# Lightbrite88/Argon_Monte_Carlo

Measured on AMD Instinct MI355X. Metric: particle-steps/sec, higher is better.
Workload: dtype f64; 1 GPU; cube_1e5; geometry=cube, n_particles=100000, n_per_gpu=100000, parallelism=single GPU

## Files before the change

### argon_monte_carlo_amd/csrc/amc_api.hip

```cpp
#include <math.h>
#include <stdarg.h>
#include <stdio.h>
#include <stdlib.h>
#include <string.h>

#include <algorithm>
#include <chrono>
#include <memory>
#include <vector>
#include <new>
#include <type_traits>

#include "amc_host.h"
#include "amc_resolve_dev.h"

int amc_fail(amc_ctx *c, int code, const char *fmt, ...)
{
    char buf[512];
    va_list ap;
    va_start(ap, fmt);
    vsnprintf(buf, sizeof buf, fmt, ap);
    va_end(ap);
    if (c) c->err = buf;
    return code;
// ... 278 lines not shown
        AMC_HIP(c, dalloc(c, &c->d_cnt, 1));
        AMC_HIP(c, hipMemsetAsync(c->d_cnt, 0, sizeof(amc_dev_counters), c->stream));
        AMC_HIP(c, dalloc(c, &c->d_banks, AMC_COUNTER_BANKS));
        AMC_HIP(c, hipMemsetAsync(c->d_banks, 0, sizeof(amc_counter_bank) * AMC_COUNTER_BANKS, c->stream));
        c->out.banks = c->d_banks;
        c->out.rec = c->d_rec; c->out.cap = (unsigned)mp; c->out.cnt = c->d_cnt;
        c->out.lo = p->hist_lo; c->out.hi = p->hist_hi;
        if (p->hist_bins > 0 && p->hist_hi > p->hist_lo) {
            const int nb = p->hist_bins;
            AMC_HIP(c, dalloc(c, &c->d_hist, (size_t)4 * nb * AMC_COUNTER_BANKS));
            AMC_HIP(c, hipMemsetAsync(c->d_hist, 0, sizeof(unsigned long long) * 4 * nb * AMC_COUNTER_BANKS, c->stream));
            AMC_HIP(c, dalloc(c, &c->d_edges, (size_t)nb + 1));
            std::vector<double> ed(nb + 1);
            const double step = (p->hist_hi - p->hist_lo) / (double)nb;
            for (int k = 0; k <= nb; k++) ed[k] = p->hist_lo + (double)k * step;
            ed[nb] = p->hist_hi;
            AMC_HIP(c, hipMemcpy(c->d_edges, ed.data(), sizeof(double) * (nb + 1), hipMemcpyHostToDevice));
            c->out.nbins = nb; c->out.hist = c->d_hist; c->out.edges = c->d_edges; c->out.bin_step = step;
        }
        {
            void *hp = nullptr, *dp = nullptr;
            if (palloc(c, &hp, 256, hipHostMallocMapped) == hipSuccess && hipHostGetDevicePointer(&dp, hp, 0) == hipSuccess) {
                memset(hp, 0, 256);
                c->h_host_ncand = (volatile int *)hp;
                c->d_host_ncand = (int *)dp;
                c->h_od_stall = (volatile int *)hp + 16; c->d_od_stall_host = (int *)dp + 16;
                c->h_od_done = (volatile int *)hp + 32; c->d_od_done_host = (int *)dp + 32;
            }
            AMC_HIP(c, dalloc(c, &c->d_od, 16));
            AMC_HIP(c, hipMemsetAsync(c->d_od, 0, 16 * sizeof(int), c->stream));
        }
        if (palloc(c, &c->h_pin, (size_t)4 << 20, hipHostMallocDefault) == hipSuccess) c->h_pin_bytes = (size_t)4 << 20;
        if (getenv("AMC_DEBUG_RESOLVE")) {
            AMC_HIP(c, dalloc(c, &c->d_dbg, 128 + 128 * 512));
            AMC_HIP(c, hipMemsetAsync(c->d_dbg, 0, sizeof(long long) * (128 + 128 * 512), c->stream));
            { const long long big = 0x7fffffffffffffffLL; AMC_HIP(c, hipMemcpyAsync(c->d_dbg + 28, &big, sizeof big, hipMemcpyHostToDevice, c->stream)); }
        }
        AMC_HIP(c, hipStreamSynchronize(c->stream));
    }
    *out = guard.release();
    return AMC_OK;
}

int amc_set_stream(amc_ctx *c, void *hip_stream)
{
    if (!c) return AMC_ERR_INVALID;
    hipSetDevice(c->device);
    amc_prof_collect(c);
    if (c->stream) hipStreamSynchronize(c->stream);
    c->stream = hip_stream ? (hipStream_t)hip_stream : c->own_stream;
    return AMC_OK;
}

int amc_use_null_stream(amc_ctx *c)
{
    if (!c) return AMC_ERR_INVALID;
    hipSetDevice(c->device);
    amc_prof_collect(c);
    if (c->stream) hipStreamSynchronize(c->stream);
    c->stream = nullptr;
    return AMC_OK;
}

int amc_synchronize(amc_ctx *c)
{
    if (!c) return AMC_ERR_INVALID;
// ... 546 lines not shown
    }
    if (n_paths) *n_paths = pending;
    if (n_collisions) *n_collisions = st.n_pp;
    c->n = n_full; c->lo = 0; c->hi = n_full;
    return rc;
}

int amc_profile(amc_ctx *c, int enable)
{
    if (!c) return AMC_ERR_INVALID;
    hipSetDevice(c->device);
    amc_prof_collect(c);
    c->profiling = enable != 0;
    return AMC_OK;
}

int amc_overlap_stats(amc_ctx *c, int64_t *out)
{
    if (!c || !out) return AMC_ERR_INVALID;
    AMC_HIP(c, hipSetDevice(c->device));
    amc_dev_counters now;
    int rc = amc_read_counters(c, &now);
    if (rc) return rc;
    out[0] = c->ovl_steps; out[1] = now.n_refiled; out[2] = c->overlap_mode; out[3] = c->max_extra;
    out[4] = c->od_ordered_launches; out[5] = c->od_steps; out[6] = c->od_stalls; out[7] = c->od_stalls_last;
    return AMC_OK;
}

int amc_kernel_times(amc_ctx *c, double *total_ms, int64_t *launches)
{
    if (!c) return AMC_ERR_INVALID;
    hipSetDevice(c->device);
    amc_prof_collect(c);
    if (c->d_dbg) {
        long long h[128];
        hipMemcpy(h, c->d_dbg, sizeof h, hipMemcpyDeviceToHost);
        const double n = h[11] > 0 ? (double)h[11] : 1.0;
        fprintf(stderr, "[amc k_resolve phases, us/launch] count-left %.1f claim %.1f | rounds: collect %.1f pairs %.1f clusters>=3: sort+load %.1f emulate %.1f | overlay %.1f validate %.1f commit %.1f | rounds %.2f cand %.1f complex-members %.2f launches %lld (idle hand-over only %lld)\n",
                h[0] / n / 100.0, h[1] / n / 100.0, h[6] / n / 100.0, h[7] / n / 100.0, h[2] / n / 100.0, h[3] / n / 100.0, h[14] / n / 100.0, h[4] / n / 100.0, h[5] / n / 100.0,
                h[8] / n, h[9] / n, h[10] / n, h[11], h[12]);
        fprintf(stderr, "[amc host candidate count] %d (what the next launch plan is chosen from)\n", c->h_host_ncand ? (int)*c->h_host_ncand : -1);
        if (h[12] > 0)
            fprintf(stderr, "[amc k_resolve idle hand-over, us/launch] entry -> counts read %.2f, -> hand-over written %.2f, -> through the barrier %.2f (%lld launches)\n",
                    h[16] / (double)h[12] / 100.0, h[17] / (double)h[12] / 100.0, h[18] / (double)h[12] / 100.0, h[12]);
        {
            std::vector<long long> wv((size_t)128 * 512);
            hipMemcpy(wv.data(), c->d_dbg + 128, sizeof(long long) * wv.size(), hipMemcpyDeviceToHost);
            long long s[128] = {0}, longest = 0;
            for (int w = 0; w < 512; w++) {
                for (int e = 3; e < 128; e++) if (e != 4) s[e] += wv[(size_t)128 * w + e];
                longest = std::max(longest, wv[(size_t)128 * w + 4]);
            }
            const double nl = h[25] > 0 ? (double)h[25] : 1.0;
            static const char *cn[8] = {"pair", "3-cluster", "4+-cluster", "not owner", "pair+again", "3-cluster+again", "4+-cluster+again", "not owner+again"};
            static const char *pn[12] = {"graph", "walk", "reserve", "small: after emulate", "pair emulate | by the wave: emulate", "publish", "grid probe", "first hop", "particles", "set-up", "overlay probe", "small: prepare"};
            fprintf(stderr, "[amc k_clusters_wide] working waves %lld in %lld launches; launch span (first working wave in -> last out) %.2f us, last out -> ordered workgroup in %.2f us, longest wave ever %.2f us\n",
                    s[3], h[25], h[27] / nl / 100.0, h[26] / nl / 100.0, longest / 100.0);
            fprintf(stderr, "[three-particle path of lane 0] %lld times, %lld continued from the pair's hit; loads + slots %.2f us, emulation %.2f us\n", s[5], s[6],
                    s[7] / (double)std::max<long long>(1, s[5]) / 100.0, s[124] / (double)std::max<long long>(1, s[5]) / 100.0);
            fprintf(stderr, "[pair-wave lifetimes, 2.5 us buckets]");
            for (int k = 0; k < 8; k++) fprintf(stderr, " %lld", s[24 + k]);
            fprintf(stderr, "\n");
            for (int k = 0; k < 8; k++) {
                if (!s[16 + k]) continue;
                fprintf(stderr, "[amc k_clusters_wide %-16s %7lld waves, %5.1f us]", cn[k], s[16 + k], s[8 + k] / (double)s[16 + k] / 100.0);
                for (int e = 0; e < 12; e++) fprintf(stderr, " %s %.2f", pn[e], s[32 + 12 * k + e] / (double)s[16 + k] / 100.0);
// ... 13 lines not shown
```

### argon_monte_carlo_amd/csrc/amc_commit_dev.h

```cpp
#pragma once
#include "amc_grid_dev.h"

#define AMC_COMMIT_BLOCKS 64

struct amc_commit_args {
    amc_resolve_ctl *ctl;
    const double4 *hist;
    int *ov_head;
    const int *ev_gen;
    const rs_event *ev;
    const int4 *sl_meta;
    const int *sl_hits;
    const uint8_t *sl_moved;
    const double *sl_state;
    int *slot_of;
    int max_slots, max_hist;
    long long lo, hi;
    int count_pp;
    int defer;
    int nogrid;
    int enabled;
    const int *od_stall;
    int od_tick;
    int from_wide;
    const int *wctl;
    int *host_ncand;
};

AMC_DEV void amc_commit_part(const amc_commit_args &C, const amc_out &O, const amc_grid &G, const amc_state &S, int gtid,
                             int gstride)
{
    amc_resolve_ctl *ctl = C.ctl;
    int c_active, c_ok, c_nslots, c_nhist, c_ncand, c_nclusters = 0, c_rounds;
    if (C.from_wide) {
        const amc_resolve_ctl *wc = (const amc_resolve_ctl *)C.wctl;
        c_ncand = wc->ncand;
        c_active = c_ncand > 0;
        c_nslots = 2 * c_ncand + wc->nslots; c_nhist = 4 * c_ncand + wc->nhist;
        c_ok = !wc->ovf; c_rounds = 1;
        if (gtid == 0) {
            for (int b = 0; b < 16; b++) c_nclusters += C.wctl[32 + b];
            if (C.host_ncand) *C.host_ncand = c_ncand;
            O.cnt->cand_count = 0;
        }
    } else {
        c_active = ctl->active; c_ok = ctl->ok && !ctl->ovf; c_nslots = ctl->nslots; c_nhist = ctl->nhist;
        c_ncand = ctl->ncand; c_rounds = ctl->rounds;
        if (gtid == 0) c_nclusters = ctl->nclusters;
    }
    if (!c_active) return;
    const bool ok = c_ok != 0;
    const bool defer = ok && C.defer;
    const int ns = c_nslots < C.max_slots ? c_nslots : C.max_slots;
    const int nh = c_nhist < C.max_hist ? c_nhist : C.max_hist;
    int my_hits = 0, my_fp = 0;
    for (int s = gtid; s < ns; s += gstride) {
        const int p = C.sl_meta[s].x;
        if (ok && C.count_pp) { const int hs = C.sl_hits[s]; my_hits += hs & 0xffff; my_fp += hs >> 16; }
        if (defer || p < 0) continue;
        if (ok && C.sl_moved[s]) {
            const double *t = C.sl_state + (size_t)s * RS_SLOT_DOUBLES;
            S.x[p] = t[0]; S.y[p] = t[1]; S.z[p] = t[2]; S.vx[p] = t[3]; S.vy[p] = t[4]; S.vz[p] = t[5];
            S.d[p] = t[6]; S.dx[p] = t[7]; S.dy[p] = t[8]; S.dz[p] = t[9]; S.flag[p] = t[10] != 0.0 ? 1 : 0;
        }
        C.slot_of[p] = -1;
    }
    for (int o = 32; o > 0; o >>= 1) { my_hits += __shfl_down(my_hits, o, 64); my_fp += __shfl_down(my_fp, o, 64); }
    if ((threadIdx.x & 63) == 0 && my_hits) atomicAdd(&O.banks[amc_bank_id()].n_pp, (unsigned long long)my_hits);
    if ((threadIdx.x & 63) == 0 && my_fp) atomicAdd(&O.banks[amc_bank_id()].n_fp_errors, (unsigned long long)my_fp);
    if (ok)
        for (int e = gtid; e < nh; e += gstride) {
            const int g = C.ev_gen[e];
            if (g == 0) continue;
            const rs_event ev = C.ev[e];
            if (g != C.sl_meta[ev.slot].z) continue;
            const int owner = ev.which ? ev.i : ev.j;
            if (owner < C.lo || owner >= C.hi) continue;
            amc_emit(O, ev.phase, ev.cell, ev.i, ev.j, ev.which, ev.val[0], ev.val[1], ev.val[2], ev.val[3]);
        }
    if (!C.nogrid)
        for (int h = gtid; h < nh; h += gstride) {
            const double4 r = C.hist[h];
// ... 14 lines not shown
```

### argon_monte_carlo_amd/csrc/amc_grid_dev.h

```cpp
#pragma once
#include "amc_internal.h"

AMC_DEV int amc_clampi(int v, int lo, int hi) { return v < lo ? lo : (v > hi ? hi : v); }

AMC_DEV void amc_grid_coords(const amc_grid &G, double x, double y, double z, int &cx, int &cy, int &cz)
{
    cx = amc_clampi((int)floor((x - G.x0) * G.inv_h), 0, G.gx - 1);
    cy = amc_clampi((int)floor((y - G.y0) * G.inv_h), 0, G.gy - 1);
    cz = amc_clampi((int)floor((z - G.z0) * G.inv_h), 0, G.gz - 1);
}

AMC_DEV int amc_grid_cell(const amc_grid &G, int cx, int cy, int cz, bool *outside)
{
    if (G.uniform) return (cz * G.gy + cy) * G.gx + cx;
    const int lo = G.lay_lo[cz], n = G.lay_n[cz];
    int lx = cx - lo, ly = cy - lo;
    if (lx < 0 || lx >= n || ly < 0 || ly >= n) {
        if (outside) *outside = true;
        lx = amc_clampi(lx, 0, n - 1);
        ly = amc_clampi(ly, 0, n - 1);
    }
    return G.lay_off[cz] + ly * n + lx;
}

// ... 32 lines not shown
    const bool ox = (fx0 < 0) || (fx0 > G.gx - 1), oy = (fy0 < 0) || (fy0 > G.gy - 1), oz = (fz0 < 0) || (fz0 > G.gz - 1);
    const int x_lo = amc_clampi(cx - ((fx < t || ox) ? 1 : 0), 0, G.gx - 1), x_hi = amc_clampi(cx + ((fx > 1.0 - t || ox) ? 1 : 0), 0, G.gx - 1);
    const int y_lo = amc_clampi(cy - ((fy < t || oy) ? 1 : 0), 0, G.gy - 1), y_hi = amc_clampi(cy + ((fy > 1.0 - t || oy) ? 1 : 0), 0, G.gy - 1);
    const int z_lo = amc_clampi(cz - ((fz < t || oz) ? 1 : 0), 0, G.gz - 1), z_hi = amc_clampi(cz + ((fz > 1.0 - t || oz) ? 1 : 0), 0, G.gz - 1);
    int run = c >> 1;
    for (int kz = z_lo; kz <= z_hi; kz++) {
        int lo = 0, nn = G.gx, off;
        if (G.uniform) off = kz * G.gy * G.gx;
        else { lo = G.lay_lo[kz]; nn = G.lay_n[kz]; off = G.lay_off[kz]; }
        const int a = amc_clampi(x_lo - lo, 0, nn - 1), b = amc_clampi(x_hi - lo, 0, nn - 1);
        const int ya = amc_clampi(y_lo - lo, 0, nn - 1), yb = amc_clampi(y_hi - lo, 0, nn - 1);
        const int ny = yb - ya + 1;
        if (run < ny) {
            const int row = off + (ya + run) * nn;
            if (c & 1) return b != a ? row + b : -1;
            return row + a;
        }
        run -= ny;
    }
    return -1;
}

AMC_DEV int amc_rec_next(const amc_rec &r) { return r.next; }
AMC_DEV int amc_node_particle(const amc_lists &B, int node) { return node < B.n ? node : B.extra[node - B.n]; }
AMC_DEV void amc_rec_pos(const amc_grid &G, const amc_rec &r, double &x, double &y, double &z)
{
    x = G.x0 + (double)r.x; y = G.y0 + (double)r.y; z = G.z0 + (double)r.z;
}
AMC_DEV int amc_list_head(const amc_lists &B, int c)
{
    const unsigned long long h = B.head[c];
    return ((unsigned int)(h >> 32) == B.epoch) ? (int)(unsigned int)(h & 0xffffffffULL) : -1;
}
AMC_DEV void amc_list_insert(const amc_grid &G, const amc_lists &B, int p, double x, double y, double z, bool *outside)
{
    amc_rec r;
    r.x = (float)(x - G.x0); r.y = (float)(y - G.y0); r.z = (float)(z - G.z0);
    double rx, ry, rz;
    amc_rec_pos(G, r, rx, ry, rz);
    int cx, cy, cz;
    amc_grid_coords(G, rx, ry, rz, cx, cy, cz);
    const int c = amc_grid_cell(G, cx, cy, cz, outside);
    const unsigned long long mine = ((unsigned long long)B.epoch << 32) | (unsigned int)p;
    const unsigned long long old = atomicExch(&B.head[c], mine);
    r.next = ((unsigned int)(old >> 32) == B.epoch) ? (int)(unsigned int)(old & 0xffffffffULL) : -1;
    B.rec[p] = r;
}

AMC_DEV int amc_list_keep(const amc_grid &G, const amc_lists &B, int p, double x, double y, double z, bool full, int wave_id,
                          int count0, int c_old, int node, bool *outside, bool *overflow)
{
    amc_rec r;
    r.x = (float)(x - G.x0); r.y = (float)(y - G.y0); r.z = (float)(z - G.z0);
    double rx, ry, rz;
    amc_rec_pos(G, r, rx, ry, rz);
    int cx, cy, cz;
    amc_grid_coords(G, rx, ry, rz, cx, cy, cz);
    const int c = amc_grid_cell(G, cx, cy, cz, outside);
    if (full) {
        const unsigned long long mine = ((unsigned long long)B.epoch << 32) | (unsigned int)p;
        const unsigned long long old = atomicExch(&B.head[c], mine);
        r.next = ((unsigned int)(old >> 32) == B.epoch) ? (int)(unsigned int)(old & 0xffffffffULL) : -1;
        B.rec[p] = r;
        B.cell_of[p] = c; B.node_of[p] = p;
        return 0;
    }
    const bool mover = c != c_old;
    const unsigned long long mv = __ballot(mover);
    if (!mover) {
        typedef float v3f_ __attribute__((ext_vector_type(3)));
        v3f_ v_; v_.x = r.x; v_.y = r.y; v_.z = r.z;
        *(v3f_ *)&B.rec[node] = v_;
        return count0 + __popcll(mv);
    }
    const int lane = (int)__lane_id();
    const int idx = count0 + __popcll(mv & ((1ULL << lane) - 1ULL));
    ((float *)&B.rec[node])[0] = __int_as_float(0x7fc00000);
    if (idx >= B.wave_cap) { *overflow = true; return count0 + __popcll(mv); }
    const int e = wave_id * B.wave_cap + idx, nn = B.n + e;
// ... 8 lines not shown
```

### argon_monte_carlo_amd/csrc/amc_internal.h

```cpp
#pragma once
#include <hip/hip_runtime.h>
#include <hip/hip_ext.h>
#include <stdint.h>

#include <string>
#include <vector>

#include "amc_device.h"

#define RS_SLOT_DOUBLES 12

struct amc_state {
    double *x, *y, *z, *vx, *vy, *vz, *d, *dx, *dy, *dz;
    double *px, *py, *pz;
    uint8_t *flag;
};

struct amc_grid {
    double x0, y0, z0, h;
    double inv_h;
    int uniform;
    int gx, gy, gz;
    int ncells;
    double cr_probe;
// ... 144 lines not shown
    int *d_lay;
    amc_lists B;
    amc_lists B_buf[2];
    int *extra_buf[2];
    int *extra_count;
    int max_extra;
    amc_wev wev_buf[2];
    hipStream_t stream2;
    hipEvent_t ev_detect, ev_stream;
    unsigned int *ovl_flags;
    unsigned int ovl_tick;
    int ovl_sync_values;
    int64_t ovl_steps;
    int keep_K;
    int lists_age = -1;
    int lists_owner;
    int overlap_mode;
    amc_resolve_ws W;
    char *w_slab;
    char *s_slab;
    amc_temp_ws T;
    amc_temp_dev_ws TD;
    amc_fields_ws F;
    bool allpairs;
    bool detect_ap;
    amc_out out;
    amc_path_record *d_rec;
    unsigned long long *d_hist;
    double *d_edges;
    amc_dev_counters *d_cnt;
    amc_counter_bank *d_banks;
    amc_dev_counters h_prev;
    long long *d_dbg;
    int cw_blocks_env;
    int stream_bs;
    int detect_bs;
    bool temp_unfused;
    bool overlap_split;
    bool profiling;
    double k_ms[AMC_K_COUNT];
    int64_t k_launches[AMC_K_COUNT];
    std::vector<std::pair<hipEvent_t, hipEvent_t>> ev_pool;
    std::vector<std::pair<int, int>> ev_pending;
    size_t ev_used;
    hipEvent_t prof_ev0, prof_ev1;
    bool mg_count_pp = true;
    volatile int *h_host_ncand;
    int *d_host_ncand;
    bool lazy_pending;
    bool commit_pending;
    bool commit_defer;
    unsigned int sweep_epoch;
    bool plan_split;
    int plan_small = AMC_PLAN_SMALL;
    char *h_pin;
    size_t h_pin_bytes;
    double *kin_send, *kin_recv;
    double *kin_vpub;
    int kin_world;
    int64_t kin_m, kin_cap, kin_block;
    int *cand_send, *cand_recv;
    int cand_cap, cand_world;
    int *mg_wave_count;
    int mg_waves_pack, mg_waves_unpack;
    bool mg_keep;
    int kin_mode = 1;
// ... 10 lines not shown
    bool od_prev_ordered = true;
    int od_tick = 1;
    int od_handled;
    int64_t od_ordered_launches;
    int64_t od_steps;
    int64_t od_stalls, od_stalls_last;
    std::vector<amc_res> owned;
};

int amc_fail(amc_ctx *c, int code, const char *fmt, ...);
#define AMC_HIP(c, call)                                                                                      \
    do {                                                                                                      \
        hipError_t e__ = (call);                                                                              \
        if (e__ != hipSuccess) return amc_fail((c), AMC_ERR_HIP, "%s failed: %s (%s:%d)", #call,             \
                                               hipGetErrorString(e__), __FILE__, __LINE__);                   \
    } while (0)

#define AMC_LAUNCH(c, kernel, grid, block, ...) \
    hipExtLaunchKernelGGL(kernel, grid, block, 0, (c)->stream, (c)->prof_ev0, (c)->prof_ev1, 0, __VA_ARGS__)
#define AMC_LAUNCH_ON(c, stream_, kernel, grid, block, ...) \
    hipExtLaunchKernelGGL(kernel, grid, block, 0, stream_, (c)->prof_ev0, (c)->prof_ev1, 0, __VA_ARGS__)

void amc_prof_begin(amc_ctx *c, int kclass);
void amc_prof_end(amc_ctx *c);
void amc_prof_cancel(amc_ctx *c);
void amc_prof_collect(amc_ctx *c);

#define AMC_ST_DRIFT 1
#define AMC_ST_WALLS 2
#define AMC_ST_BOUNDS 4
#define AMC_ST_BOUNDS_PRE 8

hipError_t amc_launch_stream(amc_ctx *c, double dt, int stages, int bounds_slot, bool fuse_bin = false);
hipError_t amc_launch_stream_ovl(amc_ctx *c, double dt, int stages, int from, unsigned int skip_epoch, hipStream_t stream,
                                 bool build_lists = true);
hipError_t amc_launch_fixup(amc_ctx *c, double dt, int stages, int from, unsigned int sweep_epoch);
hipError_t amc_launch_bin_ovl(amc_ctx *c, int to, unsigned int skip_epoch, hipStream_t stream);
hipError_t amc_launch_bin(amc_ctx *c);
hipError_t amc_launch_detect(amc_ctx *c);
hipError_t amc_launch_detect_own(amc_ctx *c);
hipError_t amc_launch_ingest(amc_ctx *c, int world);
hipError_t amc_launch_resolve(amc_ctx *c, bool defer_commit = false);
struct rs_args;
hipError_t amc_launch_wide_only(amc_ctx *c, rs_args *used);
hipError_t amc_launch_ordered(amc_ctx *c, const rs_args &used);
hipError_t amc_launch_apply(amc_ctx *c);
hipError_t amc_launch_commit(amc_ctx *c);
struct amc_commit_args;
amc_commit_args amc_make_commit_args(amc_ctx *c);
hipError_t amc_launch_temp_hits(amc_ctx *c, int case_id);
hipError_t amc_launch_temp_apply(amc_ctx *c, int case_id, int n, bool park = false);
hipError_t amc_launch_temp_velocity(amc_ctx *c, int case_id, int n);
hipError_t amc_launch_temp_cases_device(amc_ctx *c, const amc_temp_rng *cfg);
hipError_t amc_launch_kin_pack(amc_ctx *c, int world, int rank, int unpack);
int amc_kin_banks(void);
```

### argon_monte_carlo_amd/csrc/amc_stream.hip

```cpp
#include <stdlib.h>
#include <string.h>

#include <algorithm>

#include "amc_commit_dev.h"

struct amc_stream_counts {
    int nwall, nerr, noob, noob_pre;
};

template <int GEOM>
AMC_DEV void amc_stream_particle(amc_particle &q, const amc_params &P, const amc_out &O, double dt, int stages, int ip,
                                 double &px, double &py, double &pz, amc_stream_counts &cn)
{
    if ((stages & AMC_ST_BOUNDS_PRE) && GEOM != AMC_GEOM_CUBE)
        cn.noob_pre = amc_bounds(P, q.x, q.y, q.z, GEOM == AMC_GEOM_PORE_ENERGISED);
    if (stages & AMC_ST_DRIFT) {
        px = q.x; py = q.y; pz = q.z;
        const double sx = dt * q.vx, sy = dt * q.vy, sz = dt * q.vz;
        q.x += sx; q.y += sy; q.z += sz;
        q.d += fabs(sqrt(sx * sx + sy * sy + sz * sz));
        q.dx += fabs(sx); q.dy += fabs(sy); q.dz += fabs(sz);
    }
    if (stages & AMC_ST_WALLS) {
// ... 33 lines not shown
                if (amc_side_wall(q, P.R_p_c, true, O, 9, ip)) cn.nerr++; else cn.nwall++;
            }
        } else if (GEOM == AMC_GEOM_PORE_ENERGISED) {
            if (sqrt(q.x * q.x + q.y * q.y) > P.R_oa) {
                if (amc_side_wall(q, P.R_oa_c, false, O, 1, ip)) cn.nerr++;
            }
            if (q.z < 0) { const double t_ = (q.z - 0.0) / q.vz; q.vz = -q.vz; q.z = 0.0 + t_ * q.vz; }
            if (q.z > P.H) { const double t_ = (q.z - P.H) / q.vz; q.vz = -q.vz; q.z = P.H + t_ * q.vz; }
        }
    }
    if ((stages & AMC_ST_BOUNDS) && GEOM != AMC_GEOM_CUBE)
        cn.noob = amc_bounds(P, q.x, q.y, q.z, GEOM == AMC_GEOM_PORE_ENERGISED);
}

AMC_DEV void amc_stream_count(const amc_out &O, const amc_stream_counts &cn, int bounds_slot, int ip)
{
    if (!(cn.nwall | cn.nerr | cn.noob | cn.noob_pre)) return;
    if (O.wev.count) {
        amc_wev_rec r;
        r.p = ip; r.kind = 1; r.a = cn.nwall | (cn.nerr << 16); r.b = cn.noob | (cn.noob_pre << 16);
        r.v[0] = r.v[1] = r.v[2] = r.v[3] = 0.0;
        amc_wev_append(O, r);
        return;
    }
    if (cn.nwall) atomicAdd(&O.banks[amc_bank_id()].n_wall, (unsigned long long)cn.nwall);
    if (cn.nerr) atomicAdd(&O.banks[amc_bank_id()].n_fp_errors, (unsigned long long)cn.nerr);
    if (cn.noob) atomicAdd(bounds_slot ? &O.cnt->n_oob_pp : &O.cnt->n_oob_walls, (unsigned long long)cn.noob);
    if (cn.noob_pre) atomicAdd(&O.cnt->n_oob_pp, (unsigned long long)cn.noob_pre);
}

#define AMC_LD(p) __builtin_nontemporal_load(&(p))
#define AMC_ST(p, v) __builtin_nontemporal_store((v), &(p))

template <int GEOM>
__global__ __launch_bounds__(256) void k_stream(amc_state S, amc_state S_out, amc_params P, amc_out O, double dt, int stages,
                                                long long lo, long long hi, int keep_prior, int bounds_slot,
                                                amc_grid G, amc_lists B, int build_lists, amc_lazy L, amc_commit_args C,
                                                amc_ovl V)
{
    const int stalled = C.od_stall ? *C.od_stall : 0;
    if (C.enabled) {
        const unsigned nstream = gridDim.x - (unsigned)C.enabled;
        if (blockIdx.x >= nstream) {
            if (stalled && C.od_tick > stalled) return;
            amc_commit_part(C, O, G, S, (int)((blockIdx.x - nstream) * blockDim.x + threadIdx.x), (int)(C.enabled * blockDim.x));
            return;
        }
    }
    const long long p = lo + (long long)blockIdx.x * blockDim.x + threadIdx.x;
    if (p >= hi) return;
    if (V.skip_epoch && (unsigned int)(V.adj_head[p] >> 32) == V.skip_epoch) return;
    const int wave_id = (int)(blockIdx.x * (blockDim.x >> 6) + (threadIdx.x >> 6));
    const int keep_count0 = build_lists == 3 ? B.wave_count[wave_id] : 0;
    const int keep_cell = build_lists == 3 ? B.cell_of[p] : -1, keep_node = build_lists == 3 ? B.node_of[p] : (int)p;
    amc_particle q;
    q.x = AMC_LD(S.x[p]); q.y = AMC_LD(S.y[p]); q.z = AMC_LD(S.z[p]);
    q.vx = AMC_LD(S.vx[p]); q.vy = AMC_LD(S.vy[p]); q.vz = AMC_LD(S.vz[p]);
    const double x_in = q.x, y_in = q.y, z_in = q.z, vx_in = q.vx, vy_in = q.vy, vz_in = q.vz;
    const bool need_acc = (stages & (AMC_ST_DRIFT | AMC_ST_WALLS)) != 0;
    bool flag_in = false;
    double d_in = 0, dx_in = 0, dy_in = 0, dz_in = 0;
    q.d = q.dx = q.dy = q.dz = 0; q.flag = false;
    if (need_acc) {
        q.d = AMC_LD(S.d[p]); q.dx = AMC_LD(S.dx[p]); q.dy = AMC_LD(S.dy[p]); q.dz = AMC_LD(S.dz[p]);
        q.flag = S.flag[p] != 0;
        flag_in = q.flag; d_in = q.d; dx_in = q.dx; dy_in = q.dy; dz_in = q.dz;
    }
    if (stalled && C.od_tick > stalled) return;
    bool force = S_out.x != S.x;
    if (L.enabled) {
        const int sl = L.slot_of[p];
        if (sl >= 0) {
            L.slot_of[p] = -1;
            if (L.moved[sl]) {
                const double *t = L.state + (size_t)sl * RS_SLOT_DOUBLES;
                q.x = t[0]; q.y = t[1]; q.z = t[2]; q.vx = t[3]; q.vy = t[4]; q.vz = t[5];
                q.d = t[6]; q.dx = t[7]; q.dy = t[8]; q.dz = t[9]; q.flag = t[10] != 0.0;
                force = true;
            }
        }
    }
    const bool wr_acc = need_acc || force;
    double px = q.x, py = q.y, pz = q.z;
    if (!(stages & AMC_ST_DRIFT) && GEOM != AMC_GEOM_CUBE && (stages & AMC_ST_WALLS)) { px = S.px[p]; py = S.py[p]; pz = S.pz[p]; }
    amc_stream_counts cn = {0, 0, 0, 0};
    amc_stream_particle<GEOM>(q, P, O, dt, stages, (int)p, px, py, pz, cn);
    if ((stages & AMC_ST_DRIFT) && keep_prior && GEOM != AMC_GEOM_CUBE) { S.px[p] = px; S.py[p] = py; S.pz[p] = pz; }

    if (force || q.x != x_in) AMC_ST(S_out.x[p], q.x);
    if (force || q.y != y_in) AMC_ST(S_out.y[p], q.y);
    if (force || q.z != z_in) AMC_ST(S_out.z[p], q.z);
    if (force || q.vx != vx_in) S_out.vx[p] = q.vx;
    if (force || q.vy != vy_in) S_out.vy[p] = q.vy;
    if (force || q.vz != vz_in) S_out.vz[p] = q.vz;
    if (wr_acc) {
        if (force || q.d != d_in) AMC_ST(S_out.d[p], q.d);
        if (force || q.dx != dx_in) AMC_ST(S_out.dx[p], q.dx);
        if (force || q.dy != dy_in) AMC_ST(S_out.dy[p], q.dy);
        if (force || q.dz != dz_in) AMC_ST(S_out.dz[p], q.dz);
        if (force || q.flag != flag_in) S_out.flag[p] = q.flag ? 1 : 0;
    }
    if (build_lists == 1) {
        bool outside = false;
        amc_list_insert(G, B, (int)p, q.x, q.y, q.z, &outside);
        if (outside) atomicOr(&O.cnt->flags, 8ULL);
    } else if (build_lists) {
        bool outside = false, overflow = false;
        const int nc = amc_list_keep(G, B, (int)p, q.x, q.y, q.z, build_lists == 2, wave_id, keep_count0, keep_cell, keep_node, &outside, &overflow);
        if ((int)__lane_id() == __ffsll((long long)__ballot(true)) - 1) B.wave_count[wave_id] = nc;
        if (outside) atomicOr(&O.cnt->flags, 8ULL);
        if (overflow) atomicOr(&O.cnt->flags, 1ULL);
    }
    amc_stream_count(O, cn, bounds_slot, (int)p);
}

struct amc_fixup_args {
    amc_state S_in, S_out;
    amc_lists B;
    int *extra;
    int *extra_count;
    int max_extra;
    const unsigned long long *adj_head;
    const unsigned int *victim;
    unsigned int sweep_epoch;
    amc_wev wev;
    unsigned int *wev_clear;
    int *extra_clear;
    int stages, step_sweep, step_stream;
    double dt;
};

#define AMC_FIXUP_SLOT_BLOCKS 24

template <int GEOM>
__global__ __launch_bounds__(256) void k_fixup(amc_fixup_args F, amc_params P, amc_out O, amc_grid G, amc_commit_args C)
{
    if (blockIdx.x == 0 && threadIdx.x < AMC_COUNTER_BANKS) F.wev_clear[threadIdx.x] = 0;
    if (blockIdx.x == 0 && threadIdx.x == 0) *F.extra_clear = 0;
    if (F.sweep_epoch && blockIdx.x < AMC_FIXUP_SLOT_BLOCKS) {
        const int gtid = blockIdx.x * blockDim.x + threadIdx.x, gstride = AMC_FIXUP_SLOT_BLOCKS * blockDim.x;
        amc_resolve_ctl *ctl = C.ctl;
        const bool active = ctl->active != 0;
        const bool ok = ctl->ok && !ctl->ovf;
        const int ns = !active ? 0 : (ctl->nslots < C.max_slots ? ctl->nslots : C.max_slots);
        amc_out Od = O;
        Od.wev.count = nullptr;
// ... 39 lines not shown
        amc_out Os = O;
        Os.wev.count = nullptr;
        Os.step = F.step_sweep;
        amc_commit_part(C, Os, G, F.S_in, (int)((blockIdx.x - AMC_FIXUP_SLOT_BLOCKS) * blockDim.x + threadIdx.x),
                        (int)((gridDim.x - AMC_FIXUP_SLOT_BLOCKS) * blockDim.x));
    }
    amc_out Od = O;
    Od.wev.count = nullptr;
    Od.step = F.step_stream;
    for (int b = blockIdx.x; b < AMC_COUNTER_BANKS; b += gridDim.x) {
        unsigned int nb = F.wev.count[b];
        if (nb > (unsigned)F.wev.cap) nb = (unsigned)F.wev.cap;
        for (unsigned int k = threadIdx.x; k < nb; k += blockDim.x) {
            const amc_wev_rec r = F.wev.rec[(size_t)b * F.wev.cap + k];
            if (F.sweep_epoch && F.victim[r.p] == F.sweep_epoch) continue;
            if (r.kind == 0) {
                amc_emit(Od, r.a, 0, r.p, -1, 0, r.v[0], r.v[1], r.v[2], r.v[3]);
            } else {
                amc_stream_counts cn = {r.a & 0xffff, r.a >> 16, r.b & 0xffff, r.b >> 16};
                amc_stream_count(Od, cn, 0, r.p);
            }
        }
    }
}

amc_commit_args amc_make_commit_args(amc_ctx *c)
{
    const amc_resolve_ws &W = c->W;
    amc_commit_args C;
    C.ctl = (amc_resolve_ctl *)W.ctl; C.hist = W.hist; C.ov_head = W.ov_head; C.ev_gen = W.ev_gen; C.ev = W.ev;
    C.sl_meta = W.sl_meta; C.sl_hits = W.sl_hits; C.sl_moved = W.sl_moved; C.sl_state = W.sl_state; C.slot_of = W.slot_of;
    C.max_slots = W.max_slots; C.max_hist = W.max_hist; C.lo = c->lo; C.hi = c->hi; C.count_pp = c->mg_count_pp ? 1 : 0;
    C.defer = c->commit_defer ? 1 : 0; C.nogrid = c->allpairs ? 1 : 0; C.enabled = 0;
    C.od_stall = nullptr; C.od_tick = 0; C.from_wide = 0; C.wctl = nullptr; C.host_ncand = nullptr;
    return C;
}

hipError_t amc_launch_stream(amc_ctx *c, double dt, int stages, int bounds_slot, bool fuse_bin)
{
    const int threads = c->stream_bs;
    int build = 0;
    if (fuse_bin && !c->allpairs && c->lo == 0 && c->hi == c->n) {
        if (c->keep_K >= 2 && c->B.cell_of) {
            if (c->lists_owner != 1) c->lists_age = -1;
            c->lists_owner = 1;
            if (c->lists_age < 0 || c->lists_age + 1 >= c->keep_K) { build = 2; c->B.epoch++; c->lists_age = 0; }
            else { build = 3; c->lists_age++; }
        } else {
            build = 1; c->B.epoch++; c->lists_age = -1;
        }
    }
    amc_lazy L;
    memset(&L, 0, sizeof L);
    if (c->lazy_pending) {
        const amc_resolve_ws &W = c->W;
        L.slot_of = W.slot_of; L.state = W.sl_state; L.moved = W.sl_moved;
        L.enabled = 1;
        c->lazy_pending = false;
    }
    const long long cnt = c->hi - c->lo;
    if (cnt <= 0) return hipSuccess;
    amc_commit_args C = amc_make_commit_args(c);
    const amc_resolve_ws &W_ = c->W;
    unsigned extra = 0;
    if (c->commit_pending) {
        const long long lag = c->h_host_ncand ? *c->h_host_ncand : 0;
        extra = (unsigned)std::min<long long>(std::max<long long>((2 * lag + 255) / 256, 4), AMC_COMMIT_BLOCKS);
        C.enabled = (int)extra;
        c->commit_pending = false;
        if (c->od_active && !c->od_prev_ordered) { C.from_wide = 1; C.wctl = W_.wctl; C.host_ncand = c->d_host_ncand; }
    }
    if (c->od_active) { C.od_stall = c->d_od; C.od_tick = c->od_tick; }
    const unsigned blocks = (unsigned)((cnt + threads - 1) / threads) + extra;
    const int kp = c->keep_prior ? 1 : 0;
    amc_ovl V;
    V.adj_head = nullptr; V.skip_epoch = 0;
    amc_prof_begin(c, (stages == AMC_ST_BOUNDS) ? AMC_K_BOUNDS : AMC_K_DRIFT_WALLS);
    switch (c->P.geometry) {
    case AMC_GEOM_CUBE:
        AMC_LAUNCH(c, k_stream<AMC_GEOM_CUBE>, dim3(blocks), dim3(threads), c->S, c->S, c->P, c->out, dt,
                           stages, c->lo, c->hi, kp, bounds_slot, c->G, c->B, build, L, C, V);
        break;
    case AMC_GEOM_PORE:
        AMC_LAUNCH(c, k_stream<AMC_GEOM_PORE>, dim3(blocks), dim3(threads), c->S, c->S, c->P, c->out, dt,
                           stages, c->lo, c->hi, kp, bounds_slot, c->G, c->B, build, L, C, V);
        break;
    case AMC_GEOM_PORE_ENERGISED:
        AMC_LAUNCH(c, k_stream<AMC_GEOM_PORE_ENERGISED>, dim3(blocks), dim3(threads), c->S, c->S, c->P,
                           c->out, dt, stages, c->lo, c->hi, kp, bounds_slot, c->G, c->B, build, L, C, V);
        break;
    default:
        break;
    }
    amc_prof_end(c);
    return hipGetLastError();
}

hipError_t amc_launch_stream_ovl(amc_ctx *c, double dt, int stages, int from, unsigned int skip_epoch, hipStream_t stream,
                                 bool build_lists)
{
    const int to = 1 - from;
    amc_lists &Bn = c->B_buf[to];
    Bn.epoch++;
    c->lists_age = -1;
    amc_lazy L;
    memset(&L, 0, sizeof L);
    amc_commit_args C = amc_make_commit_args(c);
    amc_ovl V;
    V.adj_head = c->W.adj_head; V.skip_epoch = skip_epoch;
    amc_out O = c->out;
    O.wev = c->wev_buf[c->out.step & 1];
    const unsigned blocks = (unsigned)((c->n + 255) / 256);
    amc_prof_begin(c, AMC_K_DRIFT_WALLS);
    if (c->P.geometry == AMC_GEOM_CUBE)
        AMC_LAUNCH_ON(c, stream, k_stream<AMC_GEOM_CUBE>, dim3(blocks), dim3(256), c->S_buf[from], c->S_buf[to], c->P, O, dt, stages,
                      0LL, (long long)c->n, 0, 0, c->G, Bn, build_lists ? 1 : 0, L, C, V);
    else
        AMC_LAUNCH_ON(c, stream, k_stream<AMC_GEOM_PORE>, dim3(blocks), dim3(256), c->S_buf[from], c->S_buf[to], c->P, O, dt, stages,
                      0LL, (long long)c->n, 0, 0, c->G, Bn, build_lists ? 1 : 0, L, C, V);
    amc_prof_end(c);
    return hipGetLastError();
}

hipError_t amc_launch_fixup(amc_ctx *c, double dt, int stages, int from, unsigned int sweep_epoch)
{
    const int to = 1 - from;
    amc_fixup_args F;
    F.S_in = c->S_buf[from]; F.S_out = c->S_buf[to];
    F.B = c->B_buf[to];
    F.extra = c->extra_buf[to]; F.extra_count = c->extra_count + to; F.max_extra = c->max_extra;
    F.adj_head = c->W.adj_head; F.victim = c->W.victim; F.sweep_epoch = sweep_epoch;
    F.wev = c->wev_buf[c->out.step & 1];
    F.wev_clear = c->wev_buf[1 - (c->out.step & 1)].count;
    F.extra_clear = c->extra_count + from;
    F.stages = stages; F.step_stream = c->out.step; F.step_sweep = c->out.step - 1; F.dt = dt;
    amc_commit_args C = amc_make_commit_args(c);
    C.defer = 1;
    C.enabled = 1;
    amc_prof_begin(c, AMC_K_FIXUP);
    if (c->P.geometry == AMC_GEOM_CUBE)
        AMC_LAUNCH(c, k_fixup<AMC_GEOM_CUBE>, dim3(AMC_COMMIT_BLOCKS), dim3(256), F, c->P, c->out, c->G, C);
    else
        AMC_LAUNCH(c, k_fixup<AMC_GEOM_PORE>, dim3(AMC_COMMIT_BLOCKS), dim3(256), F, c->P, c->out, c->G, C);
    amc_prof_end(c);
    return hipGetLastError();
}
```

Before: 2.301 billion particle-steps/s.

## Reorder stream kernel loads and split list insert to overlap atomic latency

Result: no change. 2.297 billion particle-steps/s (-0.2%).

```diff
diff --git a/argon_monte_carlo_amd/csrc/amc_api.hip b/argon_monte_carlo_amd/csrc/amc_api.hip
--- a/argon_monte_carlo_amd/csrc/amc_api.hip
+++ b/argon_monte_carlo_amd/csrc/amc_api.hip
@@ -334,6 +334,10 @@
         }
         if (palloc(c, &c->h_pin, (size_t)4 << 20, hipHostMallocDefault) == hipSuccess) c->h_pin_bytes = (size_t)4 << 20;
         if (getenv("AMC_DEBUG_RESOLVE")) {
+            c->stream_dbg_waves = (size_t)n / 64 + 8 + 256;
+            AMC_HIP(c, dalloc(c, &c->d_stream_dbg, 8 * c->stream_dbg_waves));
+        }
+        if (getenv("AMC_DEBUG_RESOLVE") && atoi(getenv("AMC_DEBUG_RESOLVE")) != 2) {
             AMC_HIP(c, dalloc(c, &c->d_dbg, 128 + 128 * 512));
             AMC_HIP(c, hipMemsetAsync(c->d_dbg, 0, sizeof(long long) * (128 + 128 * 512), c->stream));
             { const long long big = 0x7fffffffffffffffLL; AMC_HIP(c, hipMemcpyAsync(c->d_dbg + 28, &big, sizeof big, hipMemcpyHostToDevice, c->stream)); }
@@ -946,6 +950,7 @@
     if (!c) return AMC_ERR_INVALID;
     hipSetDevice(c->device);
     amc_prof_collect(c);
+    amc_stream_dbg_report(c);
     if (c->d_dbg) {
         long long h[128];
         hipMemcpy(h, c->d_dbg, sizeof h, hipMemcpyDeviceToHost);
diff --git a/argon_monte_carlo_amd/csrc/amc_commit_dev.h b/argon_monte_carlo_amd/csrc/amc_commit_dev.h
--- a/argon_monte_carlo_amd/csrc/amc_commit_dev.h
+++ b/argon_monte_carlo_amd/csrc/amc_commit_dev.h
@@ -25,10 +25,11 @@
     int from_wide;
     const int *wctl;
     int *host_ncand;
+    long long *stream_dbg;
 };
 
 AMC_DEV void amc_commit_part(const amc_commit_args &C, const amc_out &O, const amc_grid &G, const amc_state &S, int gtid,
-                             int gstride)
+                             int gstride, long long *t_counts = nullptr)
 {
     amc_resolve_ctl *ctl = C.ctl;
     int c_active, c_ok, c_nslots, c_nhist, c_ncand, c_nclusters = 0, c_rounds;
@@ -48,6 +49,7 @@
         c_ncand = ctl->ncand; c_rounds = ctl->rounds;
         if (gtid == 0) c_nclusters = ctl->nclusters;
     }
+    if (t_counts) { asm volatile("s_waitcnt vmcnt(0) lgkmcnt(0)" ::: "memory"); *t_counts = wall_clock64(); }
     if (!c_active) return;
     const bool ok = c_ok != 0;
     const bool defer = ok && C.defer;
diff --git a/argon_monte_carlo_amd/csrc/amc_grid_dev.h b/argon_monte_carlo_amd/csrc/amc_grid_dev.h
--- a/argon_monte_carlo_amd/csrc/amc_grid_dev.h
+++ b/argon_monte_carlo_amd/csrc/amc_grid_dev.h
@@ -88,7 +88,7 @@
     const unsigned long long h = B.head[c];
     return ((unsigned int)(h >> 32) == B.epoch) ? (int)(unsigned int)(h & 0xffffffffULL) : -1;
 }
-AMC_DEV void amc_list_insert(const amc_grid &G, const amc_lists &B, int p, double x, double y, double z, bool *outside)
+AMC_DEV unsigned long long amc_list_push(const amc_grid &G, const amc_lists &B, int p, double x, double y, double z, bool *outside)
 {
     amc_rec r;
     r.x = (float)(x - G.x0); r.y = (float)(y - G.y0); r.z = (float)(z - G.z0);
@@ -98,9 +98,18 @@
     amc_grid_coords(G, rx, ry, rz, cx, cy, cz);
     const int c = amc_grid_cell(G, cx, cy, cz, outside);
     const unsigned long long mine = ((unsigned long long)B.epoch << 32) | (unsigned int)p;
-    const unsigned long long old = atomicExch(&B.head[c], mine);
-    r.next = ((unsigned int)(old >> 32) == B.epoch) ? (int)(unsigned int)(old & 0xffffffffULL) : -1;
-    B.rec[p] = r;
+    typedef float v3f_ __attribute__((ext_vector_type(3)));
+    v3f_ v_; v_.x = r.x; v_.y = r.y; v_.z = r.z;
+    *(v3f_ *)&B.rec[p] = v_;
+    return atomicExch(&B.head[c], mine);
+}
+AMC_DEV void amc_list_link(const amc_lists &B, int p, unsigned long long old)
+{
+    B.rec[p].next = ((unsigned int)(old >> 32) == B.epoch) ? (int)(unsigned int)(old & 0xffffffffULL) : -1;
+}
+AMC_DEV void amc_list_insert(const amc_grid &G, const amc_lists &B, int p, double x, double y, double z, bool *outside)
+{
+    amc_list_link(B, p, amc_list_push(G, B, p, x, y, z, outside));
 }
 
 AMC_DEV int amc_list_keep(const amc_grid &G, const amc_lists &B, int p, double x, double y, double z, bool full, int wave_id,
diff --git a/argon_monte_carlo_amd/csrc/amc_internal.h b/argon_monte_carlo_amd/csrc/amc_internal.h
--- a/argon_monte_carlo_amd/csrc/amc_internal.h
+++ b/argon_monte_carlo_amd/csrc/amc_internal.h
@@ -200,6 +200,12 @@
     amc_counter_bank *d_banks;
     amc_dev_counters h_prev;
     long long *d_dbg;
+    long long *d_stream_dbg;
+    size_t stream_dbg_waves;
+    std::vector<long long> h_stream_dbg;
+    std::vector<float> sdbg_phase[3][6];
+    std::vector<float> sdbg_last[3];
+    int64_t sdbg_launches, sdbg_last_kind[3];
     int cw_blocks_env;
     int stream_bs;
     int detect_bs;
@@ -276,6 +282,7 @@
 #define AMC_ST_BOUNDS_PRE 8
 
 hipError_t amc_launch_stream(amc_ctx *c, double dt, int stages, int bounds_slot, bool fuse_bin = false);
+void amc_stream_dbg_report(amc_ctx *c);
 hipError_t amc_launch_stream_ovl(amc_ctx *c, double dt, int stages, int from, unsigned int skip_epoch, hipStream_t stream,
                                  bool build_lists = true);
 hipError_t amc_launch_fixup(amc_ctx *c, double dt, int stages, int from, unsigned int sweep_epoch);
diff --git a/argon_monte_carlo_amd/csrc/amc_stream.hip b/argon_monte_carlo_amd/csrc/amc_stream.hip
--- a/argon_monte_carlo_amd/csrc/amc_stream.hip
+++ b/argon_monte_carlo_amd/csrc/amc_stream.hip
@@ -89,60 +89,84 @@
 #define AMC_LD(p) __builtin_nontemporal_load(&(p))
 #define AMC_ST(p, v) __builtin_nontemporal_store((v), &(p))
 
-template <int GEOM>
+#define ST_STAMP(k) do { if (DBG) t_st[k] = wall_clock64(); } while (0)
+#define ST_ARRIVED(k) do { if (DBG) { asm volatile("s_waitcnt vmcnt(0) lgkmcnt(0)" ::: "memory"); t_st[k] = wall_clock64(); } } while (0)
+
+template <int GEOM, bool DBG>
 __global__ __launch_bounds__(256) void k_stream(amc_state S, amc_state S_out, amc_params P, amc_out O, double dt, int stages,
                                                 long long lo, long long hi, int keep_prior, int bounds_slot,
                                                 amc_grid G, amc_lists B, int build_lists, amc_lazy L, amc_commit_args C,
                                                 amc_ovl V)
 {
+    long long t_st[8] = {0, 0, 0, 0, 0, 0, 0, 0};
+    ST_STAMP(0);
+    long long *const st_out = DBG ? C.stream_dbg + 8 * (size_t)(blockIdx.x * (blockDim.x >> 6) + (threadIdx.x >> 6)) : nullptr;
     const int stalled = C.od_stall ? *C.od_stall : 0;
-    if (C.enabled) {
-        const unsigned nstream = gridDim.x - (unsigned)C.enabled;
-        if (blockIdx.x >= nstream) {
-            if (stalled && C.od_tick > stalled) return;
-            amc_commit_part(C, O, G, S, (int)((blockIdx.x - nstream) * blockDim.x + threadIdx.x), (int)(C.enabled * blockDim.x));
-            return;
-        }
-    }
-    const long long p = lo + (long long)blockIdx.x * blockDim.x + threadIdx.x;
+    const unsigned ncommit = (unsigned)C.enabled;
+    if (blockIdx.x < ncommit) {
+        if (stalled && C.od_tick > stalled) return;
+        amc_commit_part(C, O, G, S, (int)(blockIdx.x * blockDim.x + threadIdx.x), (int)(ncommit * blockDim.x), DBG ? &t_st[1] : nullptr);
+        if (DBG) {
+            ST_ARRIVED(6);
+            if ((threadIdx.x & 63) == 0) { st_out[0] = t_st[0]; st_out[1] = t_st[1]; st_out[6] = t_st[6]; st_out[7] = 3; }
+        }
+        return;
+    }
+    const unsigned sblock = blockIdx.x - ncommit;
+    const long long p = lo + (long long)sblock * blockDim.x + threadIdx.x;
     if (p >= hi) return;
     if (V.skip_epoch && (unsigned int)(V.adj_head[p] >> 32) == V.skip_epoch) return;
-    const int wave_id = (int)(blockIdx.x * (blockDim.x >> 6) + (threadIdx.x >> 6));
+    const int sl = L.enabled ? L.slot_of[p] : -1;
+    const int wave_id = (int)(sblock * (blockDim.x >> 6) + (threadIdx.x >> 6));
     const int keep_count0 = build_lists == 3 ? B.wave_count[wave_id] : 0;
     const int keep_cell = build_lists == 3 ? B.cell_of[p] : -1, keep_node = build_lists == 3 ? B.node_of[p] : (int)p;
     amc_particle q;
     q.x = AMC_LD(S.x[p]); q.y = AMC_LD(S.y[p]); q.z = AMC_LD(S.z[p]);
     q.vx = AMC_LD(S.vx[p]); q.vy = AMC_LD(S.vy[p]); q.vz = AMC_LD(S.vz[p]);
-    const double x_in = q.x, y_in = q.y, z_in = q.z, vx_in = q.vx, vy_in = q.vy, vz_in = q.vz;
     const bool need_acc = (stages & (AMC_ST_DRIFT | AMC_ST_WALLS)) != 0;
     bool flag_in = false;
     double d_in = 0, dx_in = 0, dy_in = 0, dz_in = 0;
     q.d = q.dx = q.dy = q.dz = 0; q.flag = false;
+    unsigned int flag_raw = 0;
     if (need_acc) {
         q.d = AMC_LD(S.d[p]); q.dx = AMC_LD(S.dx[p]); q.dy = AMC_LD(S.dy[p]); q.dz = AMC_LD(S.dz[p]);
-        q.flag = S.flag[p] != 0;
-        flag_in = q.flag; d_in = q.d; dx_in = q.dx; dy_in = q.dy; dz_in = q.dz;
+        flag_raw = S.flag[p];
     }
     if (stalled && C.od_tick > stalled) return;
     bool force = S_out.x != S.x;
-    if (L.enabled) {
-        const int sl = L.slot_of[p];
-        if (sl >= 0) {
-            L.slot_of[p] = -1;
-            if (L.moved[sl]) {
-                const double *t = L.state + (size_t)sl * RS_SLOT_DOUBLES;
-                q.x = t[0]; q.y = t[1]; q.z = t[2]; q.vx = t[3]; q.vy = t[4]; q.vz = t[5];
-                q.d = t[6]; q.dx = t[7]; q.dy = t[8]; q.dz = t[9]; q.flag = t[10] != 0.0;
-                force = true;
-            }
-        }
-    }
+    bool moved = false;
+    double t_sl[11] = {0, 0, 0, 0, 0, 0, 0, 0, 0, 0, 0};
+    if (sl >= 0) {
+        const double *t = L.state + (size_t)sl * RS_SLOT_DOUBLES;
+        moved = L.moved[sl] != 0;
+#pragma unroll
+        for (int k = 0; k < 11; k++) t_sl[k] = t[k];
+        L.slot_of[p] = -1;
+    }
+    if (DBG) {
+        ST_ARRIVED(1); t_st[2] = t_st[1];
+        if (__ballot(sl >= 0)) t_st[7] = 2; else t_st[7] = 1;
+    }
+    asm volatile("" : "+v"(flag_raw));
+    q.flag = flag_raw != 0;
+    const double x_in = q.x, y_in = q.y, z_in = q.z, vx_in = q.vx, vy_in = q.vy, vz_in = q.vz;
+    if (need_acc) { flag_in = q.flag; d_in = q.d; dx_in = q.dx; dy_in = q.dy; dz_in = q.dz; }
+    q.x = moved ? t_sl[0] : q.x; q.y = moved ? t_sl[1] : q.y; q.z = moved ? t_sl[2] : q.z;
+    q.vx = moved ? t_sl[3] : q.vx; q.vy = moved ? t_sl[4] : q.vy; q.vz = moved ? t_sl[5] : q.vz;
+    q.d = moved ? t_sl[6] : q.d; q.dx = moved ? t_sl[7] : q.dx; q.dy = moved ? t_sl[8] : q.dy; q.dz = moved ? t_sl[9] : q.dz;
+    q.flag = moved ? t_sl[10] != 0.0 : q.flag;
+    force = force || moved;
     const bool wr_acc = need_acc || force;
     double px = q.x, py = q.y, pz = q.z;
     if (!(stages & AMC_ST_DRIFT) && GEOM != AMC_GEOM_CUBE && (stages & AMC_ST_WALLS)) { px = S.px[p]; py = S.py[p]; pz = S.pz[p]; }
     amc_stream_counts cn = {0, 0, 0, 0};
     amc_stream_particle<GEOM>(q, P, O, dt, stages, (int)p, px, py, pz, cn);
     if ((stages & AMC_ST_DRIFT) && keep_prior && GEOM != AMC_GEOM_CUBE) { S.px[p] = px; S.py[p] = py; S.pz[p] = pz; }
+
+    bool outside = false;
+    unsigned long long head_old = 0;
+    if (build_lists == 1) head_old = amc_list_push(G, B, (int)p, q.x, q.y, q.z, &outside);
+    ST_STAMP(3);
 
     if (force || q.x != x_in) AMC_ST(S_out.x[p], q.x);
     if (force || q.y != y_in) AMC_ST(S_out.y[p], q.y);
@@ -157,18 +181,29 @@
         if (force || q.dz != dz_in) AMC_ST(S_out.dz[p], q.dz);
         if (force || q.flag != flag_in) S_out.flag[p] = q.flag ? 1 : 0;
     }
+    ST_STAMP(4);
     if (build_lists == 1) {
-        bool outside = false;
-        amc_list_insert(G, B, (int)p, q.x, q.y, q.z, &outside);
+        ST_ARRIVED(5);
+        amc_list_link(B, (int)p, head_old);
         if (outside) atomicOr(&O.cnt->flags, 8ULL);
     } else if (build_lists) {
-        bool outside = false, overflow = false;
+        bool overflow = false;
         const int nc = amc_list_keep(G, B, (int)p, q.x, q.y, q.z, build_lists == 2, wave_id, keep_count0, keep_cell, keep_node, &outside, &overflow);
         if ((int)__lane_id() == __ffsll((long long)__ballot(true)) - 1) B.wave_count[wave_id] = nc;
         if (outside) atomicOr(&O.cnt->flags, 8ULL);
         if (overflow) atomicOr(&O.cnt->flags, 1ULL);
+        ST_ARRIVED(5);
+    } else {
+        t_st[5] = t_st[4];
     }
     amc_stream_count(O, cn, bounds_slot, (int)p);
+    if (DBG) {
+        ST_ARRIVED(6);
+        if ((int)__lane_id() == __ffsll((long long)__ballot(true)) - 1) {
+#pragma unroll
+            for (int k = 0; k < 8; k++) st_out[k] = t_st[k];
+        }
+    }
 }
 
 struct amc_fixup_args {
@@ -274,8 +309,77 @@
     C.sl_meta = W.sl_meta; C.sl_hits = W.sl_hits; C.sl_moved = W.sl_moved; C.sl_state = W.sl_state; C.slot_of = W.slot_of;
     C.max_slots = W.max_slots; C.max_hist = W.max_hist; C.lo = c->lo; C.hi = c->hi; C.count_pp = c->mg_count_pp ? 1 : 0;
     C.defer = c->commit_defer ? 1 : 0; C.nogrid = c->allpairs ? 1 : 0; C.enabled = 0;
-    C.od_stall = nullptr; C.od_tick = 0; C.from_wide = 0; C.wctl = nullptr; C.host_ncand = nullptr;
+    C.od_stall = nullptr; C.od_tick = 0; C.from_wide = 0; C.wctl = nullptr; C.host_ncand = nullptr; C.stream_dbg = nullptr;
     return C;
+}
+
+static void amc_stream_dbg_collect(amc_ctx *c, size_t waves)
+{
+    if (c->sdbg_launches >= 4096) return;
+    c->h_stream_dbg.resize(8 * waves);
+    if (hipStreamSynchronize(c->stream) != hipSuccess) return;
+    if (hipMemcpy(c->h_stream_dbg.data(), c->d_stream_dbg, sizeof(long long) * 8 * waves, hipMemcpyDeviceToHost) != hipSuccess) return;
+    long long t0 = 0, last[3] = {0, 0, 0};
+    for (size_t w = 0; w < waves; w++) {
+        const long long *t = &c->h_stream_dbg[8 * w];
+        if (t[7] >= 1 && t[7] <= 3 && (!t0 || t[0] < t0)) t0 = t[0];
+    }
+    if (!t0) return;
+    for (size_t w = 0; w < waves; w++) {
+        const long long *t = &c->h_stream_dbg[8 * w];
+        if (t[7] < 1 || t[7] > 3) continue;
+        const int k = (int)t[7] - 1;
+        if (k == 2) {
+            c->sdbg_phase[k][0].push_back((float)(t[1] - t[0]) / 100.0f);
+            c->sdbg_phase[k][1].push_back((float)(t[6] - t[1]) / 100.0f);
+        } else {
+            for (int e = 0; e < 6; e++) c->sdbg_phase[k][e].push_back((float)(t[e + 1] - t[e]) / 100.0f);
+        }
+        last[k] = std::max(last[k], t[6] - t0);
+    }
+    int lk = 0;
+    for (int k = 0; k < 3; k++) {
+        if (last[k]) c->sdbg_last[k].push_back((float)last[k] / 100.0f);
+        if (last[k] > last[lk]) lk = k;
+    }
+    c->sdbg_last_kind[lk]++;
+    c->sdbg_launches++;
+}
+
+void amc_stream_dbg_report(amc_ctx *c)
+{
+    if (!c->d_stream_dbg || !c->sdbg_launches) return;
+    auto stat = [](std::vector<float> v, double &med, double &mx) {
+        med = mx = 0;
+        if (v.empty()) return;
+        std::nth_element(v.begin(), v.begin() + v.size() / 2, v.end());
+        med = v[v.size() / 2];
+        mx = *std::max_element(v.begin(), v.end());
+    };
+    static const char *kn[3] = {"streaming", "slot_holding", "commit"};
+    static const char *pn[6] = {"entry_to_state", "state_to_slot_of", "arithmetic_exchange_issued", "to_stores_issued",
+                                "stores_to_exchange", "exchange_to_end"};
+    static const char *cpn[2] = {"entry_to_counts", "counts_to_end"};
+    fprintf(stderr, "[amc k_stream phases] {\"unit\": \"us\", \"launches\": %lld", (long long)c->sdbg_launches);
+    for (int k = 0; k < 3; k++) {
+        fprintf(stderr, ", \"%s\": {\"waves\": %zu", kn[k], c->sdbg_phase[k][0].size());
+        for (int e = 0; e < (k == 2 ? 2 : 6); e++) {
+            double med, mx;
+            stat(c->sdbg_phase[k][e], med, mx);
+            fprintf(stderr, ", \"%s\": {\"median\": %.2f, \"max\": %.2f}", k == 2 ? cpn[e] : pn[e], med, mx);
+        }
+        double med, mx;
+        stat(c->sdbg_last[k], med, mx);
+        fprintf(stderr, ", \"first_in_to_last_out\": {\"median\": %.2f, \"max\": %.2f}, \"launches_it_ended\": %lld}", med, mx,
+                (long long)c->sdbg_last_kind[k]);
+    }
+    fprintf(stderr, "}\n");
+    for (int k = 0; k < 3; k++) {
+        for (int e = 0; e < 6; e++) c->sdbg_phase[k][e].clear();
+        c->sdbg_last[k].clear();
+        c->sdbg_last_kind[k] = 0;
+    }
+    c->sdbg_launches = 0;
 }
 
 hipError_t amc_launch_stream(amc_ctx *c, double dt, int stages, int bounds_slot, bool fuse_bin)
@@ -317,24 +421,31 @@
     const int kp = c->keep_prior ? 1 : 0;
     amc_ovl V;
     V.adj_head = nullptr; V.skip_epoch = 0;
+    const size_t dbg_waves = (size_t)blocks * (size_t)(threads / 64);
+    const bool dbg = c->d_stream_dbg && (stages & AMC_ST_DRIFT) && threads % 64 == 0 && dbg_waves <= c->stream_dbg_waves;
+    if (dbg) {
+        C.stream_dbg = c->d_stream_dbg;
+        if (hipMemsetAsync(c->d_stream_dbg, 0, sizeof(long long) * 8 * dbg_waves, c->stream) != hipSuccess) return hipGetLastError();
+    }
+#define AMC_STREAM_LAUNCH(GEOM_)                                                                                              \
+    do {                                                                                                                      \
+        if (dbg)                                                                                                              \
+            AMC_LAUNCH(c, (k_stream<GEOM_, true>), dim3(blocks), dim3(threads), c->S, c->S, c->P, c->out, dt, stages, c->lo,  \
+                       c->hi, kp, bounds_slot, c->G, c->B, build, L, C, V);                                                   \
+        else                                                                                                                  \
+            AMC_LAUNCH(c, (k_stream<GEOM_, false>), dim3(blocks), dim3(threads), c->S, c->S, c->P, c->out, dt, stages, c->lo, \
+                       c->hi, kp, bounds_slot, c->G, c->B, build, L, C, V);                                                   \
+    } while (0)
     amc_prof_begin(c, (stages == AMC_ST_BOUNDS) ? AMC_K_BOUNDS : AMC_K_DRIFT_WALLS);
     switch (c->P.geometry) {
-    case AMC_GEOM_CUBE:
-        AMC_LAUNCH(c, k_stream<AMC_GEOM_CUBE>, dim3(blocks), dim3(threads), c->S, c->S, c->P, c->out, dt,
-                           stages, c->lo, c->hi, kp, bounds_slot, c->G, c->B, build, L, C, V);
-        break;
-    case AMC_GEOM_PORE:
-        AMC_LAUNCH(c, k_stream<AMC_GEOM_PORE>, dim3(blocks), dim3(threads), c->S, c->S, c->P, c->out, dt,
-                           stages, c->lo, c->hi, kp, bounds_slot, c->G, c->B, build, L, C, V);
-        break;
-    case AMC_GEOM_PORE_ENERGISED:
-        AMC_LAUNCH(c, k_stream<AMC_GEOM_PORE_ENERGISED>, dim3(blocks), dim3(threads), c->S, c->S, c->P,
-                           c->out, dt, stages, c->lo, c->hi, kp, bounds_slot, c->G, c->B, build, L, C, V);
-        break;
-    default:
-        break;
-    }
+    case AMC_GEOM_CUBE: AMC_STREAM_LAUNCH(AMC_GEOM_CUBE); break;
+    case AMC_GEOM_PORE: AMC_STREAM_LAUNCH(AMC_GEOM_PORE); break;
+    case AMC_GEOM_PORE_ENERGISED: AMC_STREAM_LAUNCH(AMC_GEOM_PORE_ENERGISED); break;
+    default: break;
+    }
+#undef AMC_STREAM_LAUNCH
     amc_prof_end(c);
+    if (dbg) amc_stream_dbg_collect(c, dbg_waves);
     return hipGetLastError();
 }
 
@@ -355,10 +466,10 @@
     const unsigned blocks = (unsigned)((c->n + 255) / 256);
     amc_prof_begin(c, AMC_K_DRIFT_WALLS);
     if (c->P.geometry == AMC_GEOM_CUBE)
-        AMC_LAUNCH_ON(c, stream, k_stream<AMC_GEOM_CUBE>, dim3(blocks), dim3(256), c->S_buf[from], c->S_buf[to], c->P, O, dt, stages,
+        AMC_LAUNCH_ON(c, stream, (k_stream<AMC_GEOM_CUBE, false>), dim3(blocks), dim3(256), c->S_buf[from], c->S_buf[to], c->P, O, dt, stages,
                       0LL, (long long)c->n, 0, 0, c->G, Bn, build_lists ? 1 : 0, L, C, V);
     else
-        AMC_LAUNCH_ON(c, stream, k_stream<AMC_GEOM_PORE>, dim3(blocks), dim3(256), c->S_buf[from], c->S_buf[to], c->P, O, dt, stages,
+        AMC_LAUNCH_ON(c, stream, (k_stream<AMC_GEOM_PORE, false>), dim3(blocks), dim3(256), c->S_buf[from], c->S_buf[to], c->P, O, dt, stages,
                       0LL, (long long)c->n, 0, 0, c->G, Bn, build_lists ? 1 : 0, L, C, V);
     amc_prof_end(c);
     return hipGetLastError();
```
